# naver/deep-image-retrieval

Hardware: AMD Instinct MI355X
Metric: images/sec descriptor extraction (resnet101-GeM, 1024x1024) (higher is better)
Workload: dtype fp16p

## Files before the change

deep-image-retrieval_amd/csrc/c_api.hip:

```cpp
#include <initializer_list>
#include <new>

#include "engine.h"
#include "pointwise.h"

namespace dir {
const char* last_error();
}
using namespace dir;

static constexpr int kSimSplitMinRows = 32768;

#define DIR_TRY try {
#define DIR_CATCH                                                   \
    }                                                               \
    catch (const std::bad_alloc&) {                                 \
        return fail(DIR_ERR_NOMEM, "out of host memory");           \
    }                                                               \
    catch (const std::exception& ex) {                              \
        return fail(DIR_ERR_INVALID, std::string("exception: ") + ex.what()); \
    }                                                               \
    catch (...) {                                                   \
        return fail(DIR_ERR_INVALID, "unknown exception");          \
    }
// ... 464 lines not shown
int dir_conv_c3c1_wpair(const void* t2, const void* w3, const void* w3_lo, const float* bias3, const void* res, void* y,
                        const void* w1, const void* w1_lo, const float* bias1, void* t1, int B, int H, int W, int P2,
                        int relu3, int relu1, void* stream) {
    DIR_TRY
    ConvArgs a;
    DIR_CHECK(fill_conv_args(a, t2, w3, bias3, res, y, B, H, W, 64, 256, 1, 1, 1, 0, H, W, relu3));
    if (!w3_lo || !w1 || !bias1 || !t1 || !res) return fail(DIR_ERR_INVALID, "conv_c3c1_wpair: null pointer");
    a.w_lo = (const uint16_t*)w3_lo;
    conv_args_next_conv1(a, (const uint16_t*)w1, (const uint16_t*)w1_lo, bias1, (uint16_t*)t1, P2, relu1 ? 1 : 0);
    if (!conv_c3c1_admissible(a))
        return fail(DIR_ERR_INVALID, "conv_c3c1_wpair: planes 64; P2 = 64 (w1_lo required) or 128 (w1_lo optional)");
    return launch_c3c1("conv_c3c1_wpair", a, DIR_FP16, stream, {t2, w3, w3_lo, res, y, w1, w1_lo, t1, bias3, bias1});
    DIR_CATCH
}

int dir_conv_c3c1_ds_wpair(const void* t2, const void* x, const void* x_lo, const void* wcat, const void* wcat_lo,
                           const float* bias, void* y, const void* w1, const void* w1_lo, const float* bias1, void* t1,
                           int B, int H, int W, int relu3, int relu1, void* stream) {
    DIR_TRY
    ConvArgs a;
    DIR_CHECK(fill_conv_args(a, t2, wcat, bias, nullptr, y, B, H, W, 64, 256, 1, 1, 1, 0, H, W, relu3));
    if (!x || !x_lo || !wcat_lo || !w1 || !w1_lo || !bias1 || !t1) return fail(DIR_ERR_INVALID, "conv_c3c1_ds_wpair: null pointer");
    a.x2 = (const uint16_t*)x;
    a.x2_lo = (const uint16_t*)x_lo;
    a.Cin2 = 64;
    a.w_lo = (const uint16_t*)wcat_lo;
    conv_args_next_conv1(a, (const uint16_t*)w1, (const uint16_t*)w1_lo, bias1, (uint16_t*)t1, 64, relu1 ? 1 : 0);
    if (!conv_c3c1_admissible(a)) return fail(DIR_ERR_INVALID, "conv_c3c1_ds_wpair: shape not admissible");
    return launch_c3c1("conv_c3c1_ds_wpair", a, DIR_FP16, stream, {t2, x, x_lo, wcat, wcat_lo, y, w1, w1_lo, t1, bias, bias1});
    DIR_CATCH
// ... 391 lines not shown
```

deep-image-retrieval_amd/csrc/conv_c3c1.hip:

```cpp
#include "dir_common.h"
#include "conv_device.h"
#include "conv_igemm.h"

namespace dir {

template <class DT, int P, bool DS, int P2, bool WP3 = false, bool WP1 = false>
__global__ void __launch_bounds__(512) conv_c3c1_kernel(const ConvArgs a) {
    static_assert(P == 64 || P == 128, "planes");
    static_assert(P2 == P || (P == 64 && P2 == 128), "conv1' width");
    static_assert(!DS || (P == 64 && P2 == 64), "the downsample form is layer1's: 64 + 64 input channels");
    static_assert((!WP3 && !WP1) || P == 64, "paired weights: layer1's seams");
    constexpr int KW = P + (DS ? 64 : 0);
    constexpr int KA = KW + (DS && WP3 ? 64 : 0);
    constexpr int C4 = 4 * P;
    constexpr int BM = 64, NT = 512;
    constexpr int CW = C4 / 8;
    constexpr int TA = CW / 32;
    constexpr int KSA = KA / 16;
    constexpr int KSW = KW / 16;
    constexpr int XBUF = BM * KA * 2;
    constexpr int NX = XBUF / 16 / NT;
    constexpr int EROW = 32 * 4 + 16;
    constexpr int EPI_OFF = 2 * XBUF;
    constexpr int OUT_OFF = EPI_OFF + 8 * 32 * EROW;
// ... 6 lines not shown
    extern __shared__ __attribute__((aligned(16))) char smem[];

    const int tid = threadIdx.x;
    const int lane = tid & 63;
    const int wave = __builtin_amdgcn_readfirstlane(tid >> 6);
    const int lrow = lane & 31, lhi = lane >> 5;

    const __amdgpu_buffer_rsrc_t rsrc_x = buffer_rsrc(a.x, a.x_bytes);
    const __amdgpu_buffer_rsrc_t rsrc_x2 =
        buffer_rsrc(DS ? a.x2 : a.x, DS ? (uint32_t)((size_t)a.M * 128) : a.x_bytes);
    const __amdgpu_buffer_rsrc_t rsrc_x2l =
        buffer_rsrc(DS && WP3 ? a.x2_lo : a.x, DS && WP3 ? (uint32_t)((size_t)a.M * 128) : a.x_bytes);
    const uint32_t y_bytes = (uint32_t)((size_t)a.M * C4 * 2);
    const uint32_t y2_bytes = (uint32_t)((size_t)a.M * P2 * 2);
    const __amdgpu_buffer_rsrc_t rsrc_r = buffer_rsrc(a.res, y_bytes);
    const __amdgpu_buffer_rsrc_t rsrc_y = buffer_rsrc(a.y, y_bytes);
    const __amdgpu_buffer_rsrc_t rsrc_y2 = buffer_rsrc(a.y2, y2_bytes);

    const int mt = (a.M + BM - 1) / BM;
    const int per = gridDim.x;
    int tile = blockIdx.x;
    if (tile >= mt) return;
    Ovf<DT> ovf;
    const int n_wave = wave * CW;

    frag_t w3[TA][KSW], w3l[WP3 ? TA : 1][WP3 ? KSW : 1];
#pragma unroll
    for (int i = 0; i < TA; ++i)
#pragma unroll
        for (int ks = 0; ks < KSW; ++ks) {
            w3[i][ks] = *(const DIR_GLOBAL frag_t*)(a.w + (size_t)(n_wave + i * 32 + lrow) * KW + ks * 16 + 8 * lhi);
// ... 52 lines not shown
    auto store_x = [&](const u32x4_t* xr, char* buf) {
#pragma unroll
        for (int i = 0; i < NX; ++i) *(u32x4_t*)(buf + i * (BM * 128) + sdst) = xr[i];
    };
    const uint32_t ncol2 = (uint32_t)((n_wave + ecol) * 2);
    auto row_off = [&](int m) { return m < a.M ? (uint32_t)m * (uint32_t)(C4 * 2) + ncol2 : kOOB; };
    auto load_res = [&](int t, int j, u32x4_t* r) {
#pragma unroll
        for (int i = 0; i < TA; ++i)
#pragma unroll
            for (int pass = 0; pass < 2; ++pass)
                r[i * 2 + pass] = __builtin_amdgcn_raw_buffer_load_b128(
                    rsrc_r, row_off(t * BM + j * 32 + pass * 16 + erow), i * 64, 0);
    };

    u32x4_t xr[NX];
    load_x(tile, xr);
    int cur = 0;
    u32x4_t rres0[TA * 2], rres1[TA * 2];
    if (!DS) load_res(tile, 0, rres0);
    store_x(xr, smem);
    __syncthreads();
    for (;;) {
        const bool more = tile + per < mt;
        const int next = more ? tile + per : tile;
        load_x(next, xr);
        const int m0 = tile * BM;
        if (!DS) load_res(tile, 1, rres1);
        const char* xb = smem + cur * XBUF;

#pragma unroll
        for (int j = 0; j < 2; ++j) {
            f32x16_t acc[TA];
#pragma unroll
            for (int i = 0; i < TA; ++i)
#pragma unroll
                for (int e = 0; e < 16; ++e) acc[i][e] = 0.f;
#pragma unroll
            for (int ks = 0; ks < KSA; ++ks) {
                const frag_t xf = *(const frag_t*)(xb + (ks >> 2) * (BM * 128) + j * (32 * 128) + lbase +
// ... 29 lines not shown
#pragma unroll
                for (int pass = 0; pass < 2; ++pass) {
                    const int mrow = pass * 16 + erow;
                    const f32x4_t f0 = *(const f32x4_t*)(ebase + mrow * EROW + ecol * 4);
                    const f32x4_t f1 = *(const f32x4_t*)(ebase + mrow * EROW + ecol * 4 + 16);
                    float v[8] = {f0[0] + b0[0], f0[1] + b0[1], f0[2] + b0[2], f0[3] + b0[3],
                                  f1[0] + b1[0], f1[1] + b1[1], f1[2] + b1[2], f1[3] + b1[3]};
                    if (!DS) {
                        const u32x4_t rv = j == 0 ? rres0[i * 2 + pass] : rres1[i * 2 + pass];
                        add_res8<DT>(v, rv);
                    }
                    if (a.relu) relu8(v);
                    u32x4_t ov;
#pragma unroll
                    for (int e = 0; e < 4; ++e) ov[e] = DT::pack(v[2 * e], v[2 * e + 1]);
                    __builtin_amdgcn_raw_buffer_store_b128(ov, rsrc_y, row_off(m0 + j * 32 + mrow), i * 64, 0);
                    ovf.see(ov);
                    const int n = n_wave + i * 32 + ecol, p = j * 32 + mrow;
                    *(u32x4_t*)(otile + (n >> 6) * (BM * 128) + p * 128 + ((((n & 63) >> 3) ^ ((p >> 1) & 7)) << 4)) = ov;
                }
                wave_lds_sync();
            }
            if (!DS && j == 0) load_res(next, 0, rres0);
        }
        __syncthreads();

        {
            constexpr int NJ = WIDE ? 2 : 1;
            f32x16_t acc1[NJ];
#pragma unroll
            for (int jj = 0; jj < NJ; ++jj)
// ... 60 lines not shown
                    ovf.see(ov);
                }
            }
        }
        if (!more) break;
        store_x(xr, smem + (cur ^ 1) * XBUF);
        tile = next;
        cur ^= 1;
        __syncthreads();
    }
    ovf.flush(a.ovf);
}

bool conv_c3c1_admissible(const ConvArgs& a) {
    const bool ds = a.x2 != nullptr;
#ifdef DIR_EXPERIMENTS
    if (a.Cin == 256) return conv_seam3_admissible(a);
#endif
    return a.R == 1 && a.S == 1 && a.stride == 1 && a.pad == 0 && a.H == a.OH && a.W == a.OW &&
           (a.Cin == 64 || a.Cin == 128) && a.Cout == 4 * a.Cin && (ds ? (a.res == nullptr && a.Cin == 64 && a.Cin2 == 64)
                                                                       : a.res != nullptr) &&
           a.w2 != nullptr && a.bias2 != nullptr && a.y2 != nullptr &&
           (a.Cout2 == a.Cin || (!ds && a.Cin == 64 && a.Cout2 == 128)) && (long)a.M * a.Cout < (1L << 30) &&
           ((!a.w_lo && !a.w2_lo && !a.x2_lo) ||
            (a.Cin == 64 && a.w_lo && (a.w2_lo || a.Cout2 == 128) && (ds ? a.x2_lo != nullptr : a.x2_lo == nullptr)));
}

template <class DT, int P, bool DS, int P2 = P, bool WP3 = false, bool WP1 = false>
static hipError_t launch_c3c1(const ConvArgs& a, hipStream_t stream) {
    constexpr int XBUF = 64 * (P + (DS ? 64 : 0) + (DS && WP3 ? 64 : 0)) * 2;
    constexpr int LDS = 2 * XBUF + 8 * 32 * (32 * 4 + 16) + 64 * 4 * P * 2 + (4 * P + P2) * 4;
    static_assert(LDS <= 160 * 1024, "LDS budget");
    auto kern = conv_c3c1_kernel<DT, P, DS, P2, WP3, WP1>;
    static std::atomic<uint64_t> attr_done{0};
    if (hipError_t e = ensure_dynamic_lds((const void*)kern, LDS, attr_done); e != hipSuccess) return e;
    ConvArgs b = a;
    b.x_bytes = (uint32_t)((size_t)a.M * a.Cin * 2);
    const int mt = (a.M + 63) / 64;
    const int ncu = cu_count();
    hipLaunchKernelGGL(kern, dim3(mt < ncu ? mt : ncu), dim3(512), LDS, stream, b);
    return hipGetLastError();
}

hipError_t conv_c3c1_launch(const ConvArgs& a, int dtype, hipStream_t stream) {
#ifdef DIR_EXPERIMENTS
    if (a.Cin == 256) return conv_seam3_launch(a, dtype, stream);
#endif
    if (a.x2 && !env().no_c3c1lc && conv_c3c1ds_lc_admissible(a)) return conv_c3c1ds_lc_launch(a, dtype, stream);
    if (a.w_lo) {
        if (dtype != DIR_FP16) return hipErrorInvalidValue;
        if (a.x2) return a.w2_lo ? launch_c3c1<FP16, 64, true, 64, true, true>(a, stream) : hipErrorInvalidValue;
        if (a.Cout2 == 128)
// ... 15 lines not shown
```

deep-image-retrieval_amd/csrc/conv_igemm.h:

```cpp
#pragma once
#include "dir_common.h"

namespace dir {

struct ConvArgs {
    const uint16_t* x;
    const uint16_t* w;
    const float* bias;
    const uint16_t* res;
    uint16_t* y;
    int B, H, W, Cin, OH, OW, Cout;
    int R, S, stride, pad, relu;
    int M;
    int Ktot;
    int T;
    int ksplit;
    float* partial;
    const uint16_t* w2;
    const float* bias2;
    uint16_t* y2;
    int Cout2, relu2;
    const uint16_t* x2;
    int Cin2;
    int H2, W2, stride2;
    uint32_t x2_bytes;
    int* ovf;
    const uint16_t* x_lo;
    const uint16_t* x2_lo;
    const uint16_t* w_lo;
    const uint16_t* w_pw;
    const uint16_t* w_s2;
    const uint16_t* w2_lo;
    const uint16_t* res_lo;
    uint16_t* y_lo;
    int tiles_m, tiles_n;
    uint32_t x_bytes, w_bytes;
// ... 145 lines not shown
```

deep-image-retrieval_amd/csrc/dir_common.h:

```cpp
#pragma once
#include <hip/hip_runtime.h>
#include <stdint.h>
#include <string.h>
#include <atomic>
#include <string>

#include "../../include/dir_engine.h"

namespace dir {

typedef __attribute__((ext_vector_type(8))) __bf16 bf16x8_t;
typedef __attribute__((ext_vector_type(8))) _Float16 f16x8_t;
typedef __attribute__((ext_vector_type(16))) float f32x16_t;
typedef __attribute__((ext_vector_type(4))) float f32x4_t;
typedef __attribute__((ext_vector_type(4))) uint32_t u32x4_t;
typedef __attribute__((ext_vector_type(2))) uint32_t u32x2_t;
typedef __attribute__((ext_vector_type(4))) int i32x4_t;
typedef __attribute__((ext_vector_type(16))) int i32x16_t;
typedef __attribute__((ext_vector_type(2))) float f32x2_t;
typedef __attribute__((ext_vector_type(2))) __bf16 bf16x2_t;
typedef __attribute__((ext_vector_type(2))) _Float16 f16x2_t;

#define DIR_GLOBAL __attribute__((address_space(1)))
#define DIR_LDS __attribute__((address_space(3)))
// ... 23 lines not shown
    bool patchw_pack = false, no_patchw_pack = false;
    bool small_k2 = false;
    bool no_patchs2 = false;
    bool x3_k2048 = false;
    bool lc1x1 = false;
    bool no_c3c1lc = false;
    bool no_smallmap = false;
    bool no_wregd = false;
    bool no_patchw_lc = false;
    bool no_xcdmap = false;
    bool no_pair_patch = false, pair_acts = false;
    int pair_stages = 1;
    bool sim_v1 = false, sim_exact = false;
    bool experiments = false;
    bool no_inplace = false;
    bool no_stem_u8 = false;
    bool stem_pair_old = false;
    bool stem_u8_prep = false;
    bool stem_u8_wg8 = false;
    int stem_u8_seg = 0;
};
const Env& env();
void reload_env();

__host__ __device__ inline uint16_t f32_to_bf16_bits(float f) {
    uint32_t u;
    memcpy(&u, &f, 4);
    if ((u & 0x7fffffffu) > 0x7f800000u) return (uint16_t)((u >> 16) | 0x40);
    u += 0x7fffu + ((u >> 16) & 1u);
    return (uint16_t)(u >> 16);
// ... 149 lines not shown
```

deep-image-retrieval_amd/csrc/engine.h:

```cpp
#pragma once
#include <map>
#include <string>
#include <vector>

#include "conv_f32.h"
#include "conv_igemm.h"
#include "pointwise.h"

namespace dir {

struct HostTensor {
    std::vector<int64_t> shape;
    std::vector<float> data;
};

struct ConvLayer {
    std::string name;
    std::string wkey;
    std::string bnprefix;
    int Cin = 0, Cout = 0, R = 1, S = 1, stride = 1, pad = 0;
    bool relu = false;
    bool stem = false;
    struct Dev {
        uint16_t* w = nullptr;
// ... 91 lines not shown
    int run_conv_f32(dir::ConvLayer& L, const float* x, const float* res, float* y, int B, int H, int W, int OH, int OW,
                     hipStream_t stream);
    int run_conv(dir::ConvLayer& L, const uint16_t* x, const uint16_t* res, uint16_t* y, int B,
                 int H, int W, int OH, int OW, hipStream_t stream, bool rev_m = false);
    int run_conv_pair(dir::ConvLayer& L, const uint16_t* x, const uint16_t* x_lo, const uint16_t* res,
                      const uint16_t* res_lo, uint16_t* y, uint16_t* y_lo, int B, int H, int W, int OH, int OW,
                      hipStream_t stream, const uint16_t* x2 = nullptr, const uint16_t* x2_lo = nullptr);
    int forward_pair_head(const void* img, int B, int H, int W, int fmt, char* base, const dir::Plan& p,
                          hipStream_t stream, uint16_t** cur, int* h, int* w, size_t* next_block);
    int forward_pair_stem(const void* img, int B, int H, int W, int fmt, char* base, const dir::Plan& p, hipStream_t stream);
    bool pick_seam(const dir::ConvLayer& c3, const dir::ConvLayer& c1, const uint16_t* t2, const uint16_t* res, uint16_t* y,
                   uint16_t* t1, int B, int H, int W, const uint16_t* block_in, const uint16_t* block_in_lo,
                   dir::ConvArgs* a) const;
    int run_seam(const dir::ConvLayer& c3, const dir::ConvLayer& c1, const dir::ConvArgs& a, hipStream_t stream);
    int pick_conv_dual(const dir::ConvLayer& c3, const dir::ConvLayer& ds, const uint16_t* t2, const uint16_t* xin,
                       uint16_t* y, int B, int Hin, int Win, int OH, int OW, dir::ConvArgs* a) const;
    int run_conv_dual(const dir::ConvLayer& c3, const dir::ConvLayer& ds, const dir::ConvArgs& a, int variant,
                      hipStream_t stream);
    int tune_conv(dir::ConvLayer& L, dir::ConvArgs& a, hipStream_t stream, int* variant);
    int finish_descriptor(float* pooled, float* fcout, int B, float* desc_out, hipStream_t stream);
    dir::Env sw;
    float* splitk_scratch = nullptr;
    bool recording() const { return profiling && !prof_paused; }
    int prof_slot(dir::ProfSlot** slot);
    template <class Label, class Launch>
    int profiled(Label&& label, double flops, double bytes, hipStream_t stream, Launch&& launch) {
        if (!recording()) return launch();
        dir::ProfSlot* s = nullptr;
        DIR_CHECK(prof_slot(&s));
        label(s->name, s->kernel);
        s->flops = flops;
// ... 15 lines not shown
```

deep-image-retrieval_amd/csrc/engine.hip:

```cpp
#include "engine.h"

#include <math.h>
#include <algorithm>

namespace dir {

static thread_local std::string g_err;
void set_error(const std::string& msg) { g_err = msg; }
int fail(int code, const std::string& msg) {
    g_err = msg;
    return code;
}
const char* last_error() { return g_err.c_str(); }


static Env read_env() {
    Env e;
    auto on = [](const char* k) { return getenv(k) != nullptr; };
    const char* mode = getenv("DIRTORCH_AMD_C3C1");
    e.c3c1_off = mode && mode[0] == '0';
    e.c3c1_force = mode && mode[0] == 'f';
    e.no_ds_seam = on("DIRTORCH_AMD_NO_DS_SEAM");
    e.no_dual = on("DIRTORCH_AMD_NO_DUAL");
    e.rev_conv1 = on("DIRTORCH_AMD_REV_CONV1");
// ... 10 lines not shown
    e.no_patchs2 = on("DIRTORCH_AMD_NO_PATCHS2");
    e.small_k2 = on("DIRTORCH_AMD_SMALL_K2");
    e.patchw_pack = on("DIRTORCH_AMD_PATCHW_PACK");
    e.no_patchw_pack = on("DIRTORCH_AMD_NO_PATCHW_PACK");
    e.no_patchw = on("DIRTORCH_AMD_NO_PATCHW");
    e.no_x3 = on("DIRTORCH_AMD_NO_X3");
    e.no_patchs = on("DIRTORCH_AMD_NO_PATCHS");
    e.no_patchw_lc = on("DIRTORCH_AMD_NO_PATCHW_LC");
    e.no_xcdmap = on("DIRTORCH_AMD_NO_XCDMAP");
    e.no_pair_patch = on("DIRTORCH_AMD_NO_PAIR_PATCH");
    e.pair_acts = on("DIRTORCH_AMD_PAIR_ACTS");
    if (const char* s = getenv("DIRTORCH_AMD_PAIR_STAGES")) e.pair_stages = atoi(s);
    e.sim_v1 = on("DIRTORCH_AMD_SIM_V1");
    e.sim_exact = on("DIRTORCH_AMD_SIM_EXACT");
    e.experiments = on("DIRTORCH_AMD_EXPERIMENTS");
    e.no_inplace = on("DIRTORCH_AMD_NO_INPLACE");
    e.no_stem_u8 = on("DIRTORCH_AMD_NO_STEM_U8");
    e.stem_u8_wg8 = on("DIRTORCH_AMD_STEM_U8_WG8");
    e.stem_u8_prep = on("DIRTORCH_AMD_STEM_U8_PREP");
    e.stem_pair_old = on("DIRTORCH_AMD_STEM_PAIR_OLD");
    if (const char* s = getenv("DIRTORCH_AMD_STEM_U8_SEG")) e.stem_u8_seg = atoi(s);
    return e;
}
static Env g_env[2];
static std::atomic<int> g_env_cur{-1};
static std::atomic_flag g_env_lock = ATOMIC_FLAG_INIT;
static void publish_env() {
    while (g_env_lock.test_and_set(std::memory_order_acquire)) {
    }
    const int cur = g_env_cur.load(std::memory_order_relaxed);
    const int nxt = cur < 0 ? 0 : 1 - cur;
// ... 612 lines not shown
        a.Cin2 = 64;
        if ((c3.dev.w_lo != nullptr) != (a.w_lo != nullptr)) return false;
    }
    conv_args_next_conv1(a, c1.dev.w, c1.dev.w_lo, c1.dev.bias, t1, c1.Cout, c1.relu ? 1 : 0);
    a.ovf = dev.ovf;
    if (c1.R != 1 || c1.S != 1 || c1.stride != 1 || c1.pad != 0 || c1.Cin != c3.Cout || !conv_c3c1_admissible(a))
        return false;
    if (!sw.c3c1_force && (a.M + 63) / 64 < (a.Cin == 256 ? kSeam3MinTiles : kSeamMinTiles)) return false;
    if (a.Cin == 256 && !sw.experiments) return false;
    return true;
}

int dir_engine::run_seam(const ConvLayer& c3, const ConvLayer& c1, const ConvArgs& a, hipStream_t stream) {
    const bool ds = a.x2 != nullptr;
    const double macs = (double)a.M * ((double)c3.Cout * (c3.Cin + a.Cin2) + (double)c1.Cout * c1.Cin);
    const double bytes = 2.0 * ((double)a.M * (c3.Cin + a.Cin2 * (a.x2_lo ? 2 : 1) + (ds ? 1.0 : 2.0) * c3.Cout + c1.Cout) +
                                (double)c3.Cout * (c3.Cin + a.Cin2) * (a.w_lo ? 2 : 1) + (double)c1.Cout * c1.Cin * (a.w2_lo ? 2 : 1));
    return profiled(
        [&](std::string& name, std::string& kernel) {
            name = c3.name.substr(0, c3.name.rfind('.')) + (ds ? ".ds+c3c1" : ".c3c1");
            kernel = (c3.Cin == 256 ? "conv_seam3<" : "conv_c3c1<") + std::to_string(c3.Cin) + (ds ? ",ds" : "") +
                     (a.w_lo ? ",wp>" : ">");
        },
        2.0 * macs, bytes, stream, [&]() -> int {
            hipError_t e = conv_c3c1_launch(a, kdtype(), stream);
            if (e != hipSuccess) return fail(DIR_ERR_HIP, std::string("conv_c3c1 launch: ") + hipGetErrorString(e));
            return DIR_OK;
        });
}

int dir_engine::pick_conv_dual(const ConvLayer& c3, const ConvLayer& ds, const uint16_t* t2, const uint16_t* xin, uint16_t* y,
                               int B, int Hin, int Win, int OH, int OW, ConvArgs* a) const {
    if (!c3.dev.w_ds || sw.no_dual || c3.dev.w_lo) return -1;
    conv_args_init(*a, {B, OH, OW, c3.Cin, c3.Cout, 1, 1, 1, 0, OH, OW, c3.relu ? 1 : 0}, t2, c3.dev.w_ds, c3.dev.bias_ds, nullptr, y);
    a->ovf = dev.ovf;
    conv_args_second_source(*a, xin, nullptr, ds.Cin);
    a->H2 = Hin;
    a->W2 = Win;
    a->stride2 = ds.stride;
    return conv_pick_dual_variant(*a);
}

int dir_engine::run_conv_dual(const ConvLayer& c3, const ConvLayer& ds, const ConvArgs& a, int variant, hipStream_t stream) {
    const double macs = (double)a.M * c3.Cout * (double)a.Ktot;
    const double bytes = 2.0 * ((double)a.M * (c3.Cin + ds.Cin + c3.Cout) + (double)c3.Cout * a.Ktot);
    return profiled(
        [&](std::string& name, std::string& kernel) {
            name = c3.name.substr(0, c3.name.rfind('.')) + ".ds+conv3";
            kernel = std::string("conv_igemm<") + conv_variant(variant).name + "/dual>";
        },
        2.0 * macs, bytes, stream, [&] { return conv_launch(a, kdtype(), variant, stream); });
}

int dir_engine::forward(const void* img, int B, int H, int W, int fmt, float* desc_out,
// ... 53 lines not shown
        } else {
            DIR_CHECK(profiled("conv1+maxpool", "stem_pool", 2.0 * B * p.OH1 * p.OW1 * 64.0 * 147.0,
                               2.0 * ((double)B * p.H2 * p.W2 * 16 + (double)B * p.PH * p.PW * 64 + 64 * 256), stream, [&] {
                                   return stem_pool_launch(s2d, convs[0].dev.w, convs[0].dev.bias, cur, B, p.H2, p.W2, p.OH1, p.OW1, kd,
                                                           stream, dev.ovf);
                               }));
        }
        h = p.PH;
        w = p.PW;
    }

    uint16_t* const pp[2] = {(uint16_t*)(base + p.bufA), (uint16_t*)(base + p.bufB)};
    uint16_t* x4 = nullptr;
    int h4 = 0, w4 = 0;
    bool t1_ready = false;
    for (size_t bi = first_block; bi < blocks.size(); ++bi) {
        BlockDef& bd = blocks[bi];
        const int oh = conv_out(h, 3, bd.stride, 1), ow = conv_out(w, 3, bd.stride, 1);
        const bool keep = (int)bi == x4_block;
        nxt = keep ? (uint16_t*)(base + p.x4) : (cur == pp[0] ? pp[1] : pp[0]);
        if (!sw.no_inplace && desc.bottleneck && bd.down < 0 && !keep && !tuning && convs[bd.conv3].Cin >= 256) nxt = cur;
        const uint16_t* resid = cur;
        const bool seam_next = desc.bottleneck && bi + 1 < blocks.size() && !tuning;
        ConvArgs seam;
        bool ds_in_seam = false;
        if (bd.down >= 0 && seam_next && !sw.no_ds_seam && convs[bd.down].Cin == 64 && convs[bd.down].stride == 1)
            ds_in_seam = pick_seam(convs[bd.conv3], convs[blocks[bi + 1].conv1], t2, nullptr, nxt, t1, B, oh, ow, cur, cur_lo, &seam);
        ConvArgs dual;
        int dual_variant = -1;
        if (bd.down >= 0 && !ds_in_seam && desc.bottleneck && !tuning && !cur_lo)
            dual_variant = pick_conv_dual(convs[bd.conv3], convs[bd.down], t2, cur, nxt, B, h, w, oh, ow, &dual);
        if (bd.down >= 0 && !ds_in_seam && dual_variant < 0) {
            DIR_CHECK(cur_lo ? run_conv_pair(convs[bd.down], cur, cur_lo, nullptr, nullptr, ds, nullptr, B, h, w, oh, ow, stream)
                             : run_conv(convs[bd.down], cur, nullptr, ds, B, h, w, oh, ow, stream));
            resid = ds;
        }
        if (desc.bottleneck) {
            if (!t1_ready)
                DIR_CHECK(cur_lo ? run_conv_pair(convs[bd.conv1], cur, cur_lo, nullptr, nullptr, t1, nullptr, B, h, w, h, w, stream)
                                 : run_conv(convs[bd.conv1], cur, nullptr, t1, B, h, w, h, w, stream, sw.rev_conv1));
            t1_ready = false;
            DIR_CHECK(run_conv(convs[bd.conv2], t1, nullptr, t2, B, h, w, oh, ow, stream));
            if (dual_variant >= 0) {
                DIR_CHECK(run_conv_dual(convs[bd.conv3], convs[bd.down], dual, dual_variant, stream));
            } else if (seam_next && (ds_in_seam || pick_seam(convs[bd.conv3], convs[blocks[bi + 1].conv1], t2, resid, nxt, t1, B, oh,
                                                             ow, nullptr, nullptr, &seam))) {
                DIR_CHECK(run_seam(convs[bd.conv3], convs[blocks[bi + 1].conv1], seam, stream));
                t1_ready = true;
            } else {
                DIR_CHECK(run_conv(convs[bd.conv3], t2, resid, nxt, B, oh, ow, oh, ow, stream, sw.rev_conv3));
            }
        } else {
            DIR_CHECK(run_conv(convs[bd.conv1], cur, nullptr, t1, B, h, w, oh, ow, stream));
            DIR_CHECK(run_conv(convs[bd.conv2], t1, resid, nxt, B, oh, ow, oh, ow, stream));
        }
        cur = nxt;
        cur_lo = nullptr;
        h = oh;
        w = ow;
        if (keep) {
            x4 = cur;
            h4 = h;
            w4 = w;
        }
    }
    if (feat_out) {
        DIR_HIP_CHECK(hipMemcpyAsync(feat_out, cur, (size_t)B * h * w * feat_dim * 2,
                                     hipMemcpyDeviceToDevice, stream));
        if (fh) *fh = h;
        if (fw) *fw = w;
        if (fc) *fc = feat_dim;
    }
// ... 137 lines not shown
```

deep-image-retrieval_amd/dirtorch_amd/_lib.py:

```python
import ctypes
import os
from ctypes import (POINTER, Structure, c_char, c_char_p, c_double, c_float, c_int, c_int64,
                    c_size_t, c_void_p)

_HERE = os.path.dirname(os.path.abspath(__file__))
LIB_PATH = os.environ.get('DIRTORCH_AMD_LIB') or os.path.join(_HERE, 'libdir_engine.so')

DIR_BF16, DIR_FP16, DIR_F32, DIR_FP16P = 0, 1, 2, 3
DIR_ERR_RANGE = -7
DTYPES = {'bf16': DIR_BF16, 'fp16': DIR_FP16, 'f32': DIR_F32, 'fp16p': DIR_FP16P}
DIR_IMG_F32_NCHW, DIR_IMG_U8_NHWC = 0, 1
DIR_POOL_GEM, DIR_POOL_MAX, DIR_POOL_AVG = 0, 1, 2
POOLING = {'gem': DIR_POOL_GEM, 'max': DIR_POOL_MAX, 'avg': DIR_POOL_AVG}
DIR_HEAD_RMAC, DIR_HEAD_FPN, DIR_HEAD_FPN0, DIR_HEAD_CLASSIFIER = 0, 1, 2, 3


class DirError(RuntimeError):

    def __init__(self, code, msg):
        super().__init__('dir_engine error %d: %s' % (code, msg))
        self.code = code


class ModelDesc(Structure):
# ... 40 lines not shown
                                    c_int, c_int, c_int, c_void_p]),
    'dir_stem_pool_pair': (c_int, [c_void_p] * 7 + [c_int] * 5 + [c_void_p]),
    'dir_stem_pool_u8': (c_int, [c_void_p] * 9 + [c_int] * 4 + [c_void_p]),
    'dir_engine_overflow': (c_int, [c_void_p, c_void_p, POINTER(c_int)]),
    'dir_conv_heuristic': (c_int, [c_int] * 12 + [c_char_p, c_int, POINTER(c_int)]),
    'dir_conv_variant_admissible': (c_int, [c_int] * 13 + [POINTER(c_int)]),
    'dir_conv_variant_splitk': (c_int, [c_int] * 13 + [POINTER(c_int)]),
    'dir_conv_bn_act_splitk': (c_int, [c_void_p, c_void_p, c_void_p, c_void_p, c_void_p] + [c_int] * 15 +
                               [c_void_p, c_size_t, POINTER(c_int), c_void_p]),
    'dir_conv_c3c1': (c_int, [c_void_p, c_void_p, c_void_p, c_void_p, c_void_p, c_void_p, c_void_p, c_void_p]
                      + [c_int] * 8 + [c_void_p]),
    'dir_conv_c3c1_ds': (c_int, [c_void_p, c_void_p, c_void_p, c_void_p, c_void_p, c_void_p, c_void_p, c_void_p]
                         + [c_int] * 6 + [c_void_p]),
    'dir_conv_c3c1_wpair': (c_int, [c_void_p] * 10 + [c_int] * 6 + [c_void_p]),
    'dir_conv_c3c1_ds_wpair': (c_int, [c_void_p] * 11 + [c_int] * 5 + [c_void_p]),
    'dir_conv_dual': (c_int, [c_void_p, c_void_p, c_void_p, c_void_p, c_void_p] + [c_int] * 11 + [c_void_p]),
    'dir_conv_bn_act_naive': (c_int, [c_void_p, c_void_p, c_void_p, c_void_p, c_void_p]
                              + [c_int] * 13 + [c_void_p]),
    'dir_prep_input': (c_int, [c_void_p, c_int, POINTER(c_float), POINTER(c_float), c_void_p,
                               c_int, c_int, c_int, c_int, c_void_p]),
    'dir_stem_pool': (c_int, [c_void_p, c_void_p, c_void_p, c_void_p, c_int, c_int, c_int, c_int, c_int,
                              c_int, c_void_p]),
    'dir_maxpool_3x3s2': (c_int, [c_void_p, c_void_p, c_int, c_int, c_int, c_int, c_int, c_void_p]),
    'dir_global_pool': (c_int, [c_void_p, c_void_p, c_int, c_int, c_int, c_int, c_int, c_float,
                                c_float, c_float, c_int, c_void_p]),
    'dir_resize_workspace_bytes': (c_int, [c_int, c_int, c_int, c_int, c_int, POINTER(c_size_t)]),
    'dir_resize_bilinear_u8': (c_int, [c_void_p, c_void_p, c_int, c_int, c_int, c_int, c_int, c_void_p,
                                       c_size_t, c_void_p]),
    'dir_upsample_add': (c_int, [c_void_p, c_void_p, c_void_p, c_int, c_int, c_int, c_int, c_int,
                                 c_int, c_int, c_void_p]),
# ... 90 lines not shown
```

deep-image-retrieval_amd/dirtorch_amd/ops.py:

```python
import ctypes

import torch

from . import _lib
from ._lib import DIR_BF16, DIR_FP16, POOLING, call, ptr, stream_ptr


def _dtype_code(t):
    if t.dtype == torch.bfloat16:
        return DIR_BF16
    if t.dtype == torch.float16:
        return DIR_FP16
    raise TypeError('16-bit activation tensor expected (bfloat16 or float16), got %s' % t.dtype)


def _need_cuda(*ts):
    for t in ts:
        if t is not None and not t.is_cuda:
            raise ValueError('device tensor expected')
        if t is not None and not t.is_contiguous():
            raise ValueError('contiguous tensor expected')


def conv_variant_names():
# ... 99 lines not shown
    return y, t1


def conv_c3c1_wpair(t2, w3, bias3, res, w1, bias1, relu3=True, relu1=True):
    (w3h, w3l), (w1h, w1l) = w3, w1
    _need_cuda(t2, w3h, w3l, bias3, res, w1h, bias1)
    B, H, W, P = t2.shape
    P2 = w1h.shape[0]
    y = torch.empty(B, H, W, 4 * P, dtype=t2.dtype, device=t2.device)
    t1 = torch.empty(B, H, W, P2, dtype=t2.dtype, device=t2.device)
    call('dir_conv_c3c1_wpair', ptr(t2), ptr(w3h), ptr(w3l), ptr(bias3), ptr(res), ptr(y), ptr(w1h),
         ptr(w1l) if w1l is not None else None, ptr(bias1), ptr(t1), B, H, W, P2, int(bool(relu3)), int(bool(relu1)), stream_ptr())
    return y, t1


def conv_c3c1_ds_wpair(t2, x, wcat, bias, w1, bias1, relu3=True, relu1=True):
    (xh, xl), (wh, wl), (w1h, w1l) = x, wcat, w1
    _need_cuda(t2, xh, xl, wh, wl, bias, w1h, w1l, bias1)
    B, H, W, P = t2.shape
    y = torch.empty(B, H, W, 256, dtype=t2.dtype, device=t2.device)
    t1 = torch.empty(B, H, W, 64, dtype=t2.dtype, device=t2.device)
    call('dir_conv_c3c1_ds_wpair', ptr(t2), ptr(xh), ptr(xl), ptr(wh), ptr(wl), ptr(bias), ptr(y), ptr(w1h), ptr(w1l),
         ptr(bias1), ptr(t1), B, H, W, int(bool(relu3)), int(bool(relu1)), stream_ptr())
    return y, t1


def conv_dual(t2, x, wcat, bias, stride2=2, relu=True):
    _need_cuda(t2, x, wcat, bias)
    B, OH, OW, Cin = t2.shape
    _, H2, W2, Cin2 = x.shape
# ... 549 lines not shown
```

include/dir_engine.h:

```cpp
#ifndef DIR_ENGINE_H
#define DIR_ENGINE_H

#include <stddef.h>
#include <stdint.h>

#ifdef __cplusplus
extern "C" {
#endif

typedef enum dir_status {
    DIR_OK = 0,
    DIR_ERR_INVALID = -1,
    DIR_ERR_STATE = -2,
    DIR_ERR_MISSING = -3,
    DIR_ERR_WORKSPACE = -4,
    DIR_ERR_HIP = -5,
    DIR_ERR_NOMEM = -6,
    DIR_ERR_RANGE = -7
} dir_status;

typedef enum dir_dtype {
    DIR_BF16 = 0,
    DIR_FP16 = 1,
    DIR_F32 = 2,
// ... 100 lines not shown
                           size_t scratch_bytes, int* ksplit_used, void* stream);
int dir_conv_c3c1(const void* t2, const void* w3, const float* bias3, const void* res, void* y, const void* w1,
                  const float* bias1, void* t1, int B, int H, int W, int P, int P2, int relu3, int relu1, int dtype,
                  void* stream);
int dir_conv_dual(const void* t2, const void* x, const void* wcat, const float* bias, void* y, int B, int OH, int OW,
                  int Cin, int Cout, int Cin2, int H2, int W2, int stride2, int relu, int dtype, void* stream);
int dir_conv_c3c1_ds(const void* t2, const void* x, const void* wcat, const float* bias, void* y, const void* w1,
                     const float* bias1, void* t1, int B, int H, int W, int relu3, int relu1, int dtype,
                     void* stream);
int dir_conv_c3c1_wpair(const void* t2, const void* w3, const void* w3_lo, const float* bias3, const void* res, void* y,
                        const void* w1, const void* w1_lo, const float* bias1, void* t1, int B, int H, int W, int P2,
                        int relu3, int relu1, void* stream);
int dir_conv_c3c1_ds_wpair(const void* t2, const void* x, const void* x_lo, const void* wcat, const void* wcat_lo,
                           const float* bias, void* y, const void* w1, const void* w1_lo, const float* bias1, void* t1,
                           int B, int H, int W, int relu3, int relu1, void* stream);
int dir_conv_bn_act_naive(const void* x, const void* w, const float* bias, const void* res,
                          void* y, int B, int H, int W, int Cin, int Cout, int R, int S,
                          int stride, int pad, int OH, int OW, int relu, int dtype, void* stream);
int dir_prep_input(const void* img, int img_format, const float* mean3, const float* std3,
                   void* out, int B, int H, int W, int dtype, void* stream);
int dir_stem_pool(const void* s2d, const void* w, const float* bias, void* y, int B, int H2, int W2,
                  int OH, int OW, int dtype, void* stream);
int dir_resize_workspace_bytes(int B, int H, int W, int OH, int OW, size_t* bytes);
int dir_resize_bilinear_u8(const void* src, void* dst, int B, int H, int W, int OH, int OW,
                           void* workspace, size_t workspace_bytes, void* stream);
int dir_maxpool_3x3s2(const void* x, void* y, int B, int H, int W, int C, int dtype, void* stream);
int dir_global_pool(const void* x, float* out, int B, int H, int W, int C, int pooling, float p,
                    float eps, float center_bias, int dtype, void* stream);
int dir_upsample_add(const void* x, const void* low, void* y, int B, int H, int W, int h, int w, int C,
                     int dtype, void* stream);
// ... 60 lines not shown
```

Measured before the change: 2445.

## Store only stride-2-kept pixels of the last block before a downsample stage

When the next bottleneck block downsamples with a 1x1 stride-2 projection, the fused conv3+conv1 seam kernel now writes its block output only at even (oh, ow) positions into a compact tensor. The next block's dual conv then reads that compact input with stride 1. This removes three quarters of that output's global writes and shrinks the downsample read, at the cost of per-row index division in the epilogue. A tile-order rotation spreads the kept rows across workgroups, and a new env switch adds low-channel in-place reuse.

```diff
diff --git a/deep-image-retrieval_amd/csrc/c_api.hip b/deep-image-retrieval_amd/csrc/c_api.hip
--- a/deep-image-retrieval_amd/csrc/c_api.hip
+++ b/deep-image-retrieval_amd/csrc/c_api.hip
@@ -502,6 +502,27 @@
     DIR_CATCH
 }
 
+int dir_conv_c3c1_sub(const void* t2, const void* w3, const void* w3_lo, const float* bias3, const void* res, void* y,
+                      const void* w1, const void* w1_lo, const float* bias1, void* t1, int B, int H, int W, int P, int P2,
+                      int relu3, int relu1, int dtype, int y_sub, int* ovf, void* stream) {
+    DIR_TRY
+    ConvArgs a;
+    DIR_CHECK(fill_conv_args(a, t2, w3, bias3, res, y, B, H, W, P, 4 * P, 1, 1, 1, 0, H, W, relu3));
+    if (!w1 || !bias1 || !t1 || !res) return fail(DIR_ERR_INVALID, "conv_c3c1_sub: null pointer");
+    if (dtype != DIR_BF16 && dtype != DIR_FP16) return fail(DIR_ERR_INVALID, "conv_c3c1_sub: bad dtype");
+    if (y_sub < 0 || y_sub > 2) return fail(DIR_ERR_INVALID, "conv_c3c1_sub: y_sub must be 0, 1 or 2");
+    if (((uintptr_t)ovf & 3) != 0) return fail(DIR_ERR_INVALID, "conv_c3c1_sub: misaligned overflow word");
+    a.w_lo = (const uint16_t*)w3_lo;
+    a.y_sub = y_sub;
+    a.ovf = ovf;
+    conv_args_next_conv1(a, (const uint16_t*)w1, (const uint16_t*)w1_lo, bias1, (uint16_t*)t1, P2, relu1 ? 1 : 0);
+    if (!conv_c3c1_admissible(a))
+        return fail(DIR_ERR_INVALID, "conv_c3c1_sub: planes 64 (P2 = 64 or 128) or 128 (P2 = 128); paired weights as dir_conv_c3c1_wpair; "
+                                     "with y_sub = 2 the compact y must not overlap res");
+    return launch_c3c1("conv_c3c1_sub", a, dtype, stream, {t2, w3, w3_lo, res, y, w1, w1_lo, t1, bias3, bias1});
+    DIR_CATCH
+}
+
 int dir_conv_c3c1_ds_wpair(const void* t2, const void* x, const void* x_lo, const void* wcat, const void* wcat_lo,
                            const float* bias, void* y, const void* w1, const void* w1_lo, const float* bias1, void* t1,
                            int B, int H, int W, int relu3, int relu1, void* stream) {
diff --git a/deep-image-retrieval_amd/csrc/conv_c3c1.hip b/deep-image-retrieval_amd/csrc/conv_c3c1.hip
--- a/deep-image-retrieval_amd/csrc/conv_c3c1.hip
+++ b/deep-image-retrieval_amd/csrc/conv_c3c1.hip
@@ -4,9 +4,10 @@
 
 namespace dir {
 
-template <class DT, int P, bool DS, int P2, bool WP3 = false, bool WP1 = false>
+template <class DT, int P, bool DS, int P2, bool WP3 = false, bool WP1 = false, bool SUB = false>
 __global__ void __launch_bounds__(512) conv_c3c1_kernel(const ConvArgs a) {
     static_assert(P == 64 || P == 128, "planes");
+    static_assert(!SUB || !DS, "the compact store: non-DS forms");
     static_assert(P2 == P || (P == 64 && P2 == 128), "conv1' width");
     static_assert(!DS || (P == 64 && P2 == 64), "the downsample form is layer1's: 64 + 64 input channels");
     static_assert((!WP3 && !WP1) || P == 64, "paired weights: layer1's seams");
@@ -44,7 +45,8 @@
     const uint32_t y_bytes = (uint32_t)((size_t)a.M * C4 * 2);
     const uint32_t y2_bytes = (uint32_t)((size_t)a.M * P2 * 2);
     const __amdgpu_buffer_rsrc_t rsrc_r = buffer_rsrc(a.res, y_bytes);
-    const __amdgpu_buffer_rsrc_t rsrc_y = buffer_rsrc(a.y, y_bytes);
+    const int OHc = (a.OH + 1) >> 1, OWc = (a.OW + 1) >> 1;
+    const __amdgpu_buffer_rsrc_t rsrc_y = buffer_rsrc(a.y, SUB ? (uint32_t)((size_t)a.B * OHc * OWc * C4 * 2) : y_bytes);
     const __amdgpu_buffer_rsrc_t rsrc_y2 = buffer_rsrc(a.y2, y2_bytes);
 
     const int mt = (a.M + BM - 1) / BM;
@@ -127,6 +129,16 @@
                     rsrc_r, row_off(t * BM + j * 32 + pass * 16 + erow), i * 64, 0);
     };
 
+    auto sub_off = [&](int m) {
+        const uint32_t mm = m < a.M ? (uint32_t)m : 0u;
+        const uint32_t b = fast_div(mm, a.div_ohw_mul, a.div_ohw_shr);
+        const uint32_t rem = mm - b * (uint32_t)(a.OH * a.OW);
+        const uint32_t oh = fast_div(rem, a.div_ow_mul, a.div_ow_shr);
+        const uint32_t ow = rem - oh * (uint32_t)a.OW;
+        const bool kept = m < a.M && ((oh | ow) & 1u) == 0;
+        return kept ? ((b * (uint32_t)OHc + (oh >> 1)) * (uint32_t)OWc + (ow >> 1)) * (uint32_t)(C4 * 2) + ncol2 : kOOB;
+    };
+
     u32x4_t xr[NX];
     load_x(tile, xr);
     int cur = 0;
@@ -134,9 +146,22 @@
     if (!DS) load_res(tile, 0, rres0);
     store_x(xr, smem);
     __syncthreads();
+    int slot = blockIdx.x, round_base = 0;
+    int shift = 0;
+    if (SUB) {
+        const int tpr = (a.OW + BM - 1) / BM;
+        shift = (((per * BM) / a.OW) & 1) == 0 && tpr < per ? tpr : 0;
+    }
     for (;;) {
-        const bool more = tile + per < mt;
-        const int next = more ? tile + per : tile;
+        int next_tile = tile + per;
+        if (SUB) {
+            slot += shift;
+            if (slot >= per) slot -= per;
+            round_base += per;
+            next_tile = round_base + slot;
+        }
+        const bool more = next_tile < mt;
+        const int next = more ? next_tile : tile;
         load_x(next, xr);
         const int m0 = tile * BM;
         if (!DS) load_res(tile, 1, rres1);
@@ -196,7 +221,11 @@
                     u32x4_t ov;
 #pragma unroll
                     for (int e = 0; e < 4; ++e) ov[e] = DT::pack(v[2 * e], v[2 * e + 1]);
-                    __builtin_amdgcn_raw_buffer_store_b128(ov, rsrc_y, row_off(m0 + j * 32 + mrow), i * 64, 0);
+                    if constexpr (SUB) {
+                        __builtin_amdgcn_raw_buffer_store_b128(ov, rsrc_y, sub_off(m0 + j * 32 + mrow), i * 64, 0);
+                    } else {
+                        __builtin_amdgcn_raw_buffer_store_b128(ov, rsrc_y, row_off(m0 + j * 32 + mrow), i * 64, 0);
+                    }
                     ovf.see(ov);
                     const int n = n_wave + i * 32 + ecol, p = j * 32 + mrow;
                     *(u32x4_t*)(otile + (n >> 6) * (BM * 128) + p * 128 + ((((n & 63) >> 3) ^ ((p >> 1) & 7)) << 4)) = ov;
@@ -287,6 +316,11 @@
 
 bool conv_c3c1_admissible(const ConvArgs& a) {
     const bool ds = a.x2 != nullptr;
+    if (a.y_sub < 0 || a.y_sub > 2) return false;
+    if (a.y_sub == 2) {
+        const size_t full = (size_t)a.M * a.Cout, compact = (size_t)a.B * ((a.OH + 1) / 2) * ((a.OW + 1) / 2) * a.Cout;
+        if (ds || a.Cin == 256 || !a.res || !a.y || (a.y < a.res + full && a.res < a.y + compact)) return false;
+    }
 #ifdef DIR_EXPERIMENTS
     if (a.Cin == 256) return conv_seam3_admissible(a);
 #endif
@@ -299,16 +333,23 @@
             (a.Cin == 64 && a.w_lo && (a.w2_lo || a.Cout2 == 128) && (ds ? a.x2_lo != nullptr : a.x2_lo == nullptr)));
 }
 
-template <class DT, int P, bool DS, int P2 = P, bool WP3 = false, bool WP1 = false>
+template <class DT, int P, bool DS, int P2 = P, bool WP3 = false, bool WP1 = false, bool SUB = false>
 static hipError_t launch_c3c1(const ConvArgs& a, hipStream_t stream) {
+    if constexpr (!DS && !SUB) {
+        if (a.y_sub == 2) return launch_c3c1<DT, P, DS, P2, WP3, WP1, true>(a, stream);
+    }
     constexpr int XBUF = 64 * (P + (DS ? 64 : 0) + (DS && WP3 ? 64 : 0)) * 2;
     constexpr int LDS = 2 * XBUF + 8 * 32 * (32 * 4 + 16) + 64 * 4 * P * 2 + (4 * P + P2) * 4;
     static_assert(LDS <= 160 * 1024, "LDS budget");
-    auto kern = conv_c3c1_kernel<DT, P, DS, P2, WP3, WP1>;
+    auto kern = conv_c3c1_kernel<DT, P, DS, P2, WP3, WP1, SUB>;
     static std::atomic<uint64_t> attr_done{0};
     if (hipError_t e = ensure_dynamic_lds((const void*)kern, LDS, attr_done); e != hipSuccess) return e;
     ConvArgs b = a;
     b.x_bytes = (uint32_t)((size_t)a.M * a.Cin * 2);
+    if (SUB) {
+        fastdiv_init((uint32_t)(a.OH * a.OW), b.div_ohw_mul, b.div_ohw_shr);
+        fastdiv_init((uint32_t)a.OW, b.div_ow_mul, b.div_ow_shr);
+    }
     const int mt = (a.M + 63) / 64;
     const int ncu = cu_count();
     hipLaunchKernelGGL(kern, dim3(mt < ncu ? mt : ncu), dim3(512), LDS, stream, b);
diff --git a/deep-image-retrieval_amd/csrc/conv_igemm.h b/deep-image-retrieval_amd/csrc/conv_igemm.h
--- a/deep-image-retrieval_amd/csrc/conv_igemm.h
+++ b/deep-image-retrieval_amd/csrc/conv_igemm.h
@@ -20,6 +20,7 @@
     const float* bias2;
     uint16_t* y2;
     int Cout2, relu2;
+    int y_sub;
     const uint16_t* x2;
     int Cin2;
     int H2, W2, stride2;
diff --git a/deep-image-retrieval_amd/csrc/dir_common.h b/deep-image-retrieval_amd/csrc/dir_common.h
--- a/deep-image-retrieval_amd/csrc/dir_common.h
+++ b/deep-image-retrieval_amd/csrc/dir_common.h
@@ -61,6 +61,8 @@
     bool sim_v1 = false, sim_exact = false;
     bool experiments = false;
     bool no_inplace = false;
+    bool no_inplace_low = false;
+    bool no_prune = false;
     bool no_stem_u8 = false;
     bool stem_pair_old = false;
     bool stem_u8_prep = false;
diff --git a/deep-image-retrieval_amd/csrc/engine.h b/deep-image-retrieval_amd/csrc/engine.h
--- a/deep-image-retrieval_amd/csrc/engine.h
+++ b/deep-image-retrieval_amd/csrc/engine.h
@@ -129,7 +129,7 @@
                    dir::ConvArgs* a) const;
     int run_seam(const dir::ConvLayer& c3, const dir::ConvLayer& c1, const dir::ConvArgs& a, hipStream_t stream);
     int pick_conv_dual(const dir::ConvLayer& c3, const dir::ConvLayer& ds, const uint16_t* t2, const uint16_t* xin,
-                       uint16_t* y, int B, int Hin, int Win, int OH, int OW, dir::ConvArgs* a) const;
+                       uint16_t* y, int B, int Hin, int Win, int OH, int OW, dir::ConvArgs* a, bool xin_compact = false) const;
     int run_conv_dual(const dir::ConvLayer& c3, const dir::ConvLayer& ds, const dir::ConvArgs& a, int variant,
                       hipStream_t stream);
     int tune_conv(dir::ConvLayer& L, dir::ConvArgs& a, hipStream_t stream, int* variant);
diff --git a/deep-image-retrieval_amd/csrc/engine.hip b/deep-image-retrieval_amd/csrc/engine.hip
--- a/deep-image-retrieval_amd/csrc/engine.hip
+++ b/deep-image-retrieval_amd/csrc/engine.hip
@@ -48,7 +48,10 @@
     e.sim_v1 = on("DIRTORCH_AMD_SIM_V1");
     e.sim_exact = on("DIRTORCH_AMD_SIM_EXACT");
     e.experiments = on("DIRTORCH_AMD_EXPERIMENTS");
-    e.no_inplace = on("DIRTORCH_AMD_NO_INPLACE");
+    const char* inplace = getenv("DIRTORCH_AMD_NO_INPLACE");
+    e.no_inplace_low = inplace && inplace[0] == 'l';
+    e.no_inplace = inplace && !e.no_inplace_low;
+    e.no_prune = on("DIRTORCH_AMD_NO_PRUNE");
     e.no_stem_u8 = on("DIRTORCH_AMD_NO_STEM_U8");
     e.stem_u8_wg8 = on("DIRTORCH_AMD_STEM_U8_WG8");
     e.stem_u8_prep = on("DIRTORCH_AMD_STEM_U8_PREP");
@@ -691,7 +694,8 @@
 int dir_engine::run_seam(const ConvLayer& c3, const ConvLayer& c1, const ConvArgs& a, hipStream_t stream) {
     const bool ds = a.x2 != nullptr;
     const double macs = (double)a.M * ((double)c3.Cout * (c3.Cin + a.Cin2) + (double)c1.Cout * c1.Cin);
-    const double bytes = 2.0 * ((double)a.M * (c3.Cin + a.Cin2 * (a.x2_lo ? 2 : 1) + (ds ? 1.0 : 2.0) * c3.Cout + c1.Cout) +
+    const double ypix = a.y_sub == 2 ? (double)a.B * ((a.OH + 1) / 2) * ((a.OW + 1) / 2) : (double)a.M;
+    const double bytes = 2.0 * ((double)a.M * (c3.Cin + a.Cin2 * (a.x2_lo ? 2 : 1) + (ds ? 0.0 : 1.0) * c3.Cout + c1.Cout) + ypix * c3.Cout +
                                 (double)c3.Cout * (c3.Cin + a.Cin2) * (a.w_lo ? 2 : 1) + (double)c1.Cout * c1.Cin * (a.w2_lo ? 2 : 1));
     return profiled(
         [&](std::string& name, std::string& kernel) {
@@ -707,14 +711,14 @@
 }
 
 int dir_engine::pick_conv_dual(const ConvLayer& c3, const ConvLayer& ds, const uint16_t* t2, const uint16_t* xin, uint16_t* y,
-                               int B, int Hin, int Win, int OH, int OW, ConvArgs* a) const {
+                               int B, int Hin, int Win, int OH, int OW, ConvArgs* a, bool xin_compact) const {
     if (!c3.dev.w_ds || sw.no_dual || c3.dev.w_lo) return -1;
     conv_args_init(*a, {B, OH, OW, c3.Cin, c3.Cout, 1, 1, 1, 0, OH, OW, c3.relu ? 1 : 0}, t2, c3.dev.w_ds, c3.dev.bias_ds, nullptr, y);
     a->ovf = dev.ovf;
     conv_args_second_source(*a, xin, nullptr, ds.Cin);
-    a->H2 = Hin;
-    a->W2 = Win;
-    a->stride2 = ds.stride;
+    a->H2 = xin_compact ? OH : Hin;
+    a->W2 = xin_compact ? OW : Win;
+    a->stride2 = xin_compact ? 1 : ds.stride;
     return conv_pick_dual_variant(*a);
 }
 
@@ -798,22 +802,41 @@
     uint16_t* x4 = nullptr;
     int h4 = 0, w4 = 0;
     bool t1_ready = false;
+    bool cur_compact = false;
     for (size_t bi = first_block; bi < blocks.size(); ++bi) {
         BlockDef& bd = blocks[bi];
         const int oh = conv_out(h, 3, bd.stride, 1), ow = conv_out(w, 3, bd.stride, 1);
         const bool keep = (int)bi == x4_block;
         nxt = keep ? (uint16_t*)(base + p.x4) : (cur == pp[0] ? pp[1] : pp[0]);
-        if (!sw.no_inplace && desc.bottleneck && bd.down < 0 && !keep && !tuning && convs[bd.conv3].Cin >= 256) nxt = cur;
+        ConvArgs seam;
+        bool prune = false;
+        if (!sw.no_prune && desc.bottleneck && bd.down < 0 && !keep && !tuning && bi + 1 < blocks.size() && blocks[bi + 1].down >= 0) {
+            const BlockDef& nb = blocks[bi + 1];
+            const ConvLayer& nds = convs[nb.down];
+            ConvArgs probe;
+            prune = nds.R == 1 && nds.S == 1 && nds.stride == 2 && nds.pad == 0 && nb.stride == 2 &&
+                    pick_seam(convs[bd.conv3], convs[nb.conv1], t2, cur, nxt, t1, B, oh, ow, nullptr, nullptr, &seam) &&
+                    pick_conv_dual(convs[nb.conv3], nds, t2, nxt, cur, B, oh, ow, conv_out(oh, 3, 2, 1), conv_out(ow, 3, 2, 1), &probe,
+                                   true) >= 0;
+            if (prune) {
+                seam.y_sub = 2;
+                prune = conv_c3c1_admissible(seam);
+            }
+        }
+        if (!prune && !sw.no_inplace && desc.bottleneck && bd.down < 0 && !keep && !tuning &&
+            (convs[bd.conv3].Cin >= 256 || !sw.no_inplace_low))
+            nxt = cur;
         const uint16_t* resid = cur;
         const bool seam_next = desc.bottleneck && bi + 1 < blocks.size() && !tuning;
-        ConvArgs seam;
         bool ds_in_seam = false;
         if (bd.down >= 0 && seam_next && !sw.no_ds_seam && convs[bd.down].Cin == 64 && convs[bd.down].stride == 1)
             ds_in_seam = pick_seam(convs[bd.conv3], convs[blocks[bi + 1].conv1], t2, nullptr, nxt, t1, B, oh, ow, cur, cur_lo, &seam);
         ConvArgs dual;
         int dual_variant = -1;
         if (bd.down >= 0 && !ds_in_seam && desc.bottleneck && !tuning && !cur_lo)
-            dual_variant = pick_conv_dual(convs[bd.conv3], convs[bd.down], t2, cur, nxt, B, h, w, oh, ow, &dual);
+            dual_variant = pick_conv_dual(convs[bd.conv3], convs[bd.down], t2, cur, nxt, B, h, w, oh, ow, &dual, cur_compact);
+        if (cur_compact && (dual_variant < 0 || !t1_ready))
+            return fail(DIR_ERR_STATE, "forward: a pruned block output without its two-source reader");
         if (bd.down >= 0 && !ds_in_seam && dual_variant < 0) {
             DIR_CHECK(cur_lo ? run_conv_pair(convs[bd.down], cur, cur_lo, nullptr, nullptr, ds, nullptr, B, h, w, oh, ow, stream)
                              : run_conv(convs[bd.down], cur, nullptr, ds, B, h, w, oh, ow, stream));
@@ -827,8 +850,8 @@
             DIR_CHECK(run_conv(convs[bd.conv2], t1, nullptr, t2, B, h, w, oh, ow, stream));
             if (dual_variant >= 0) {
                 DIR_CHECK(run_conv_dual(convs[bd.conv3], convs[bd.down], dual, dual_variant, stream));
-            } else if (seam_next && (ds_in_seam || pick_seam(convs[bd.conv3], convs[blocks[bi + 1].conv1], t2, resid, nxt, t1, B, oh,
-                                                             ow, nullptr, nullptr, &seam))) {
+            } else if (seam_next && (ds_in_seam || prune || pick_seam(convs[bd.conv3], convs[blocks[bi + 1].conv1], t2, resid, nxt, t1, B,
+                                                                      oh, ow, nullptr, nullptr, &seam))) {
                 DIR_CHECK(run_seam(convs[bd.conv3], convs[blocks[bi + 1].conv1], seam, stream));
                 t1_ready = true;
             } else {
@@ -840,6 +863,7 @@
         }
         cur = nxt;
         cur_lo = nullptr;
+        cur_compact = prune;
         h = oh;
         w = ow;
         if (keep) {
diff --git a/deep-image-retrieval_amd/dirtorch_amd/_lib.py b/deep-image-retrieval_amd/dirtorch_amd/_lib.py
--- a/deep-image-retrieval_amd/dirtorch_amd/_lib.py
+++ b/deep-image-retrieval_amd/dirtorch_amd/_lib.py
@@ -78,6 +78,7 @@
                          + [c_int] * 6 + [c_void_p]),
     'dir_conv_c3c1_wpair': (c_int, [c_void_p] * 10 + [c_int] * 6 + [c_void_p]),
     'dir_conv_c3c1_ds_wpair': (c_int, [c_void_p] * 11 + [c_int] * 5 + [c_void_p]),
+    'dir_conv_c3c1_sub': (c_int, [c_void_p] * 10 + [c_int] * 9 + [c_void_p, c_void_p]),
     'dir_conv_dual': (c_int, [c_void_p, c_void_p, c_void_p, c_void_p, c_void_p] + [c_int] * 11 + [c_void_p]),
     'dir_conv_bn_act_naive': (c_int, [c_void_p, c_void_p, c_void_p, c_void_p, c_void_p]
                               + [c_int] * 13 + [c_void_p]),
diff --git a/deep-image-retrieval_amd/dirtorch_amd/ops.py b/deep-image-retrieval_amd/dirtorch_amd/ops.py
--- a/deep-image-retrieval_amd/dirtorch_amd/ops.py
+++ b/deep-image-retrieval_amd/dirtorch_amd/ops.py
@@ -137,6 +137,26 @@
     return y, t1
 
 
+def conv_c3c1_sub(t2, w3, bias3, res, w1, bias1, y_sub=2, relu3=True, relu1=True, y=None, ovf=None):
+    (w3h, w3l) = w3 if isinstance(w3, tuple) else (w3, None)
+    (w1h, w1l) = w1 if isinstance(w1, tuple) else (w1, None)
+    _need_cuda(t2, w3h, w3l, bias3, res, w1h, w1l, bias1, y, ovf)
+    B, H, W, P = t2.shape
+    P2 = w1h.shape[0]
+    oh, ow = ((H + 1) // 2, (W + 1) // 2) if y_sub == 2 else (H, W)
+    if y is None:
+        y = torch.empty(B, oh, ow, 4 * P, dtype=t2.dtype, device=t2.device)
+    elif y.dtype != t2.dtype or y.numel() < B * oh * ow * 4 * P:
+        raise ValueError('y: %d elements of %s expected' % (B * oh * ow * 4 * P, t2.dtype))
+    if ovf is not None and (ovf.dtype != torch.int32 or ovf.numel() != 1):
+        raise TypeError('ovf: one int32 element expected')
+    t1 = torch.empty(B, H, W, P2, dtype=t2.dtype, device=t2.device)
+    call('dir_conv_c3c1_sub', ptr(t2), ptr(w3h), ptr(w3l) if w3l is not None else None, ptr(bias3), ptr(res), ptr(y), ptr(w1h),
+         ptr(w1l) if w1l is not None else None, ptr(bias1), ptr(t1), B, H, W, P, P2, int(bool(relu3)), int(bool(relu1)),
+         _dtype_code(t2), int(y_sub), ptr(ovf) if ovf is not None else None, stream_ptr())
+    return y, t1
+
+
 def conv_c3c1_ds_wpair(t2, x, wcat, bias, w1, bias1, relu3=True, relu1=True):
     (xh, xl), (wh, wl), (w1h, w1l) = x, wcat, w1
     _need_cuda(t2, xh, xl, wh, wl, bias, w1h, w1l, bias1)
diff --git a/include/dir_engine.h b/include/dir_engine.h
--- a/include/dir_engine.h
+++ b/include/dir_engine.h
@@ -138,6 +138,9 @@
 int dir_conv_c3c1_ds_wpair(const void* t2, const void* x, const void* x_lo, const void* wcat, const void* wcat_lo,
                            const float* bias, void* y, const void* w1, const void* w1_lo, const float* bias1, void* t1,
                            int B, int H, int W, int relu3, int relu1, void* stream);
+int dir_conv_c3c1_sub(const void* t2, const void* w3, const void* w3_lo, const float* bias3, const void* res, void* y,
+                      const void* w1, const void* w1_lo, const float* bias1, void* t1, int B, int H, int W, int P, int P2,
+                      int relu3, int relu1, int dtype, int y_sub, int* ovf, void* stream);
 int dir_conv_bn_act_naive(const void* x, const void* w, const float* bias, const void* res,
                           void* y, int B, int H, int W, int Cin, int Cout, int R, int S,
                           int stride, int pad, int OH, int OW, int relu, int dtype, void* stream);
```

New measurement: 2458, median of 6. About the same (+0.5%).
